# deeppowers/deeppowers

Measured on NVIDIA H100. Metric: ct_mult_relin_per_s, higher is better.
Workload: dtype u64

## Files before the change

deeppowers_b200/csrc/kernels.cu:

```cuda
#include <cooperative_groups.h>
#include <cuda.h>
#include <cuda_runtime.h>

#include <atomic>

#include "kernel_bodies.cuh"
#include "launch_util.hpp"

#ifndef DPFHE_PART
#define DPFHE_PART 0
#endif
#define DPFHE_PART_MAIN (DPFHE_PART == 0 || DPFHE_PART == 1)
#define DPFHE_PART_HYBRID (DPFHE_PART == 0 || DPFHE_PART == 2)
#define DPFHE_PART_GROUPED (DPFHE_PART == 0 || DPFHE_PART == 3)

namespace dpfhe {
namespace DPFHE_VNS {

__device__ __forceinline__ u32 ld_acquire_u32(const u32 *p) {
    u32 v;
    asm volatile("ld.acquire.gpu.global.u32 %0, [%1];" : "=r"(v) : "l"(p) : "memory");
    return v;
}
__device__ __forceinline__ void st_release_u32(u32 *p, u32 v) {
    asm volatile("st.release.gpu.global.u32 [%0], %1;" ::"l"(p), "r"(v) : "memory");
}
__device__ __forceinline__ u64 ld_acquire_u64(const u64 *p) {
    u64 v;
    asm volatile("ld.acquire.gpu.global.u64 %0, [%1];" : "=l"(v) : "l"(p) : "memory");
    return v;
}
__device__ __forceinline__ void st_release_u64(u64 *p, u64 v) {
    asm volatile("st.release.gpu.global.u64 [%0], %1;" ::"l"(p), "l"(v) : "memory");
}
__device__ __forceinline__ void spin_until(const u32 *flag, u32 tag) {
    while ((int)(ld_acquire_u32(flag) - tag) < 0) {
    }
}
__device__ __forceinline__ void wait_flags(const u32 *flags, u32 count, u32 tag) {
    if (threadIdx.x < count) spin_until(flags + threadIdx.x, tag);
    __syncthreads();
}
__device__ __forceinline__ void publish_flag(u32 *flag, u32 tag) {
    __threadfence();
    __syncthreads();
    if (threadIdx.x == 0) st_release_u32(flag, tag);
}
template <class Box>
__device__ __forceinline__ u32 draw_ticket(u32 *ticket, Box box, u32 tag, bool leader, bool post) {
    __shared__ u32 s_ct;
    if (threadIdx.x == 0) {
        u64 *const mb = box();
        if (leader) {
            const u32 t = atomicAdd(ticket, 1u);
            if (post) st_release_u64(mb, ((u64)tag << 32) | t);
            s_ct = t;
        } else {
            u64 m;
            do m = ld_acquire_u64(mb);
            while ((u32)(m >> 32) != tag);
            s_ct = (u32)m;
        }
    }
    __syncthreads();
    return s_ct;
}

template <int NT, bool PROF = false>
struct DevCta {
    unsigned long long *prof = nullptr;
    long long last = 0;
    unsigned long long t_start = 0, c_start = 0;
    __device__ __forceinline__ void prof_begin(unsigned long long *all) {
        if (PROF) {
            prof = all + (size_t)blockIdx.x * 16;
            last = clock64();
            c_start = (unsigned long long)last;
            asm volatile("mov.u64 %0, %%globaltimer;" : "=l"(t_start));
        }
    }
    __device__ __forceinline__ void prof_end() {
        if (PROF && threadIdx.x == 0) {
            unsigned long long t_end;
            asm volatile("mov.u64 %0, %%globaltimer;" : "=l"(t_end));
            prof[14] += t_end - t_start;
            prof[15] += (unsigned long long)clock64() - c_start;
        }
    }
    __device__ __forceinline__ void mark(int id) {
        if (PROF && threadIdx.x == 0) {
            const long long now = clock64();
            prof[id] += (unsigned long long)(now - last);
            last = now;
        }
    }
    template <class F>
    __device__ __forceinline__ void par(F f) {
        f((int)threadIdx.x);
        __syncthreads();
    }
    __device__ __forceinline__ void wait_ge(const u32 *flag, u32 target) { wait_flags(flag, 1, target); }
    template <class F>
    __device__ __forceinline__ void par_dom(F f) {
        f((int)threadIdx.x);
        if (NT <= 256) __syncthreads();
        else asm volatile("bar.sync %0, 256;" ::"r"(1 + ((int)threadIdx.x >> 8)) : "memory");
    }
    template <class F>
    __device__ __forceinline__ void par_warp(F f) {
        f((int)threadIdx.x);
        __syncwarp();
    }
};

#if DPFHE_PART_MAIN
template <int LOGN, int NT, int MINB, bool INVERSE>
__global__ void __launch_bounds__(NT, MINB) ntt_kernel(u64 *data, const Twiddle *__restrict__ tables,
                                                        const __grid_constant__ LimbTable lt, u32 L, size_t n_limbs) {
    extern __shared__ __align__(1024) unsigned char smem_raw[];
    u64 *buf = reinterpret_cast<u64 *>(smem_raw);
    constexpr size_t N = (size_t)1 << LOGN;
    DevCta<NT> cta;
    for (size_t w = blockIdx.x; w < n_limbs; w += gridDim.x) {
        const u32 l = (u32)(w % L);
        const LimbParams &p = lt.lp[l];
        if (INVERSE) ntt_inv_body<LOGN, NT>(cta, buf, data + w * N, tables + (size_t)l * N, p);
        else ntt_fwd_body<LOGN, NT>(cta, buf, data + w * N, tables + (size_t)l * N, p);
    }
}

__device__ __forceinline__ u32 smem_addr(const void *p) { return (u32)__cvta_generic_to_shared(p); }

template <int LOGN, int NT, int MINB>
__global__ void __launch_bounds__(NT, MINB) ntt_inv_tma_kernel(const __grid_constant__ CUtensorMap tm, u64 *data, const Twiddle *__restrict__ itw,
                                                                const __grid_constant__ LimbTable lt, u32 L) {
    extern __shared__ __align__(1024) unsigned char smem_raw[];
    __shared__ __align__(8) unsigned long long bar;
    u64 *buf = reinterpret_cast<u64 *>(smem_raw);
    constexpr size_t N = (size_t)1 << LOGN;
    constexpr int ROWS = (int)(N * 8 / 128), BOX_ROWS = ROWS < 256 ? ROWS : 256, BOXES = ROWS / BOX_ROWS;
    DevCta<NT> cta;
    const size_t w = blockIdx.x;
    const u32 l = (u32)(w % L);
    const u32 bar_a = smem_addr(&bar);
    if (threadIdx.x == 0) {
        asm volatile("mbarrier.init.shared::cta.b64 [%0], 1;" ::"r"(bar_a) : "memory");
        asm volatile("fence.mbarrier_init.release.cluster;" ::: "memory");
    }
    __syncthreads();
    if (threadIdx.x == 0) {
        asm volatile("mbarrier.arrive.expect_tx.shared::cta.b64 _, [%0], %1;" ::"r"(bar_a), "r"((u32)(N * 8)) : "memory");
#pragma unroll
        for (int b = 0; b < BOXES; ++b) {
            const int row = (int)(w * ROWS) + b * BOX_ROWS;
            asm volatile("cp.async.bulk.tensor.2d.shared::cluster.global.mbarrier::complete_tx::bytes [%0], [%1, {%2, %3}], [%4];"
                         ::"r"(smem_addr(smem_raw + (size_t)b * BOX_ROWS * 128)), "l"(reinterpret_cast<unsigned long long>(&tm)), "r"(0), "r"(row), "r"(bar_a)
                         : "memory");
        }
    }
    {
        u32 done = 0;
        while (!done) {
            asm volatile("{\n\t.reg .pred p;\n\tmbarrier.try_wait.parity.shared::cta.b64 p, [%1], 0;\n\tselp.u32 %0, 1, 0, p;\n\t}"
                         : "=r"(done)
                         : "r"(bar_a)
                         : "memory");
        }
    }
    ntt_inv_resident<LOGN, NT>(cta, buf, data + w * N, itw + (size_t)l * N, lt.lp[l]);
}

template <int NT, int MINB, bool INVERSE>
__global__ void __cluster_dims__(2, 1, 1) __launch_bounds__(NT, MINB)
    ntt_pair_kernel(u64 *data, const Twiddle *__restrict__ tables, const __grid_constant__ LimbTable lt, u32 L, size_t n_limbs) {
    extern __shared__ __align__(1024) unsigned char smem_raw[];
    u64 *buf = reinterpret_cast<u64 *>(smem_raw);
    constexpr size_t N = (size_t)1 << NTT_PAIR_LOGN;
    namespace cg = cooperative_groups;
    cg::cluster_group cluster = cg::this_cluster();
    const int h = (int)cluster.block_rank();
    const u64 *peer = cluster.map_shared_rank(buf, h ^ 1);
    DevCta<NT> cta;
    for (size_t w = blockIdx.x / 2; w < n_limbs; w += gridDim.x / 2) {
        const u32 l = (u32)(w % L);
        const LimbParams &p = lt.lp[l];
        const Twiddle *tw = tables + (size_t)l * N;
        if (!INVERSE) {
            ntt_fwd_half_load<NT>(cta, buf, data + w * N, tw, p, h);
            cluster.sync();
            ntt_fwd_half_finish<NT>(cta, buf, data + w * N, tw, p, h);
        } else {
            ntt_inv_half_passes<NT>(cta, buf, data + w * N, tw, p, h);
            cluster.sync();
            ntt_inv_half_outer<NT>(cta, buf, peer, data + w * N, tw, p, h);
            cluster.sync();
        }
    }
}

template <int LOGN, int NT, int MINB>
__global__ void __launch_bounds__(NT, MINB) ms_tau_kernel(const u64 *in, u64 *tau, const Twiddle *__restrict__ itw,
                                                           const __grid_constant__ LimbTable lt, const __grid_constant__ MsConsts K,
                                                           u32 L, size_t n_polys) {
    extern __shared__ __align__(1024) unsigned char smem_raw[];
    u64 *buf = reinterpret_cast<u64 *>(smem_raw);
    constexpr size_t N = (size_t)1 << LOGN;
    DevCta<NT> cta;
    const LimbParams &p = lt.lp[L - 1];
    for (size_t w = blockIdx.x; w < n_polys; w += gridDim.x)
        ms_tau_body<LOGN, NT>(cta, buf, in + (w * L + (L - 1)) * N, nullptr, itw + (size_t)(L - 1) * N, p, tau + w * N, K);
}

template <int LOGN, int NT, int MINB>
__global__ void __launch_bounds__(NT, MINB) ms_limb_kernel(const u64 *in, const u64 *tau, u64 *out, const Twiddle *__restrict__ tw,
                                                            const __grid_constant__ LimbTable lt, const __grid_constant__ MsConsts K,
                                                            u32 L, size_t n_items) {
    extern __shared__ __align__(1024) unsigned char smem_raw[];
    u64 *buf = reinterpret_cast<u64 *>(smem_raw);
    constexpr size_t N = (size_t)1 << LOGN;
    DevCta<NT> cta;
    const u32 Lo = L - 1;
    for (size_t w = blockIdx.x; w < n_items; w += gridDim.x) {
        const size_t poly = w / Lo;
        const u32 i = (u32)(w % Lo);
        ms_limb_body<LOGN, NT>(cta, buf, tau + poly * N, in + (poly * L + i) * N, out + (poly * Lo + i) * N, tw + (size_t)i * N, lt.lp[i], K, i);
    }
}

template <int LOGN, int NT, int MINB>
__global__ void __launch_bounds__(NT, MINB) md_tau_kernel(const u64 *in, u64 *tau, const Twiddle *__restrict__ itw, const __grid_constant__ MsConsts K,
                                                           const __grid_constant__ GroupConsts G, size_t n_items) {
    extern __shared__ __align__(1024) unsigned char smem_raw[];
    u64 *buf = reinterpret_cast<u64 *>(smem_raw);
    constexpr size_t N = (size_t)1 << LOGN;
    DevCta<NT> cta;
    const u32 L = G.Lq + G.K;
    for (size_t w = blockIdx.x; w < n_items; w += gridDim.x) {
        const size_t poly = w / G.K;
        const u32 s = G.Lq + (u32)(w % G.K);
        ms_tau_body<LOGN, NT>(cta, buf, in + (poly * L + s) * N, nullptr, itw + (size_t)s * N, G.lp_up[s], tau + w * N, K);
    }
}

template <int LOGN, int NT, int MINB>
__global__ void __launch_bounds__(NT, MINB) md_limb_kernel(const u64 *in, const u64 *tau, u64 *out, const Twiddle *__restrict__ tw,
                                                            const __grid_constant__ LimbTable lt, const __grid_constant__ MsConsts K,
                                                            const __grid_constant__ GroupConsts G, size_t n_items) {
    extern __shared__ __align__(1024) unsigned char smem_raw[];
    u64 *buf = reinterpret_cast<u64 *>(smem_raw);
    constexpr size_t N = (size_t)1 << LOGN;
    DevCta<NT> cta;
    const u32 Lq = G.Lq, L = Lq + G.K;
    for (size_t w = blockIdx.x; w < n_items; w += gridDim.x) {
        const size_t poly = w / Lq;
        const u32 i = (u32)(w % Lq);
        ms_limb_group<LOGN, NT, false>(cta, buf, tau + poly * G.K * N, N, in + (poly * L + i) * N, out + (poly * Lq + i) * N, tw + (size_t)i * N,
                                       lt.lp[i], K, G, i);
    }
}

template <int LOGN, int NT>
__global__ void __launch_bounds__(NT, 1) ckks_enc_fft_kernel(const Cplx *slots, double *coeffs, const Cplx *__restrict__ tw,
                                                              const u32 *__restrict__ tj, double sc) {
    extern __shared__ __align__(1024) unsigned char smem_raw[];
    constexpr size_t N = (size_t)1 << LOGN;
    DevCta<NT> cta;
    const size_t v = blockIdx.x;
    ckks_enc_fft_body<LOGN, NT>(cta, reinterpret_cast<Cplx *>(smem_raw), slots + v * (N / 2), coeffs + v * N, tw, tj, sc);
}

template <int LOGN, int NT, int MINB>
__global__ void __launch_bounds__(NT, MINB) ckks_enc_ntt_kernel(const double *coeffs, u64 *pt, const Twiddle *__restrict__ tw,
                                                                 const u64 *__restrict__ pow2, const __grid_constant__ LimbTable lt, u32 L) {
    extern __shared__ __align__(1024) unsigned char smem_raw[];
    u64 *buf = reinterpret_cast<u64 *>(smem_raw);
    constexpr size_t N = (size_t)1 << LOGN;
    DevCta<NT> cta;
    const size_t w = blockIdx.x;
    const u32 l = (u32)(w % L);
    const LimbParams &p = lt.lp[l];
    const double *x = coeffs + (w / L) * N;
    const u64 *p2 = pow2 + (size_t)l * CKKS_POW2_E;
    auto src = [&](int c) {
        U64x2 r;
        r.x = ckks_reduce(x[2 * c], p, p2);
        r.y = ckks_reduce(x[2 * c + 1], p, p2);
        return r;
    };
    ntt_fwd_src_body<LOGN, NT>(cta, buf, src, pt + w * N, tw + (size_t)l * N, p);
}

template <int NT, int MINB>
__global__ void __launch_bounds__(NT, MINB) ckks_enc_ntt_pair_kernel(const double *coeffs, u64 *pt, const Twiddle *__restrict__ tw,
                                                                      const u64 *__restrict__ pow2, const __grid_constant__ LimbTable lt, u32 L) {
    extern __shared__ __align__(1024) unsigned char smem_raw[];
    u64 *buf = reinterpret_cast<u64 *>(smem_raw);
    constexpr size_t N = (size_t)1 << NTT_PAIR_LOGN;
    DevCta<NT> cta;
    const size_t w = blockIdx.x / 2;
    const int h = (int)(blockIdx.x & 1);
    const u32 l = (u32)(w % L);
    const LimbParams &p = lt.lp[l];
    const double *x = coeffs + (w / L) * N;
    const u64 *p2 = pow2 + (size_t)l * CKKS_POW2_E;
    auto src = [&](int c) {
        U64x2 r;
        r.x = ckks_reduce(x[2 * c], p, p2);
        r.y = ckks_reduce(x[2 * c + 1], p, p2);
        return r;
    };
    ntt_fwd_half_load_src<NT>(cta, buf, src, tw + (size_t)l * N, p, h);
    ntt_fwd_half_finish<NT>(cta, buf, pt + w * N, tw + (size_t)l * N, p, h);
}

template <int LOGN, int NT>
__global__ void __launch_bounds__(NT, 1) ckks_dec_kernel(u64 *work, Cplx *slots, const Cplx *__restrict__ tw, const u32 *__restrict__ tj,
                                                          const __grid_constant__ LimbTable lt, const __grid_constant__ CkksConsts K, u32 L) {
    extern __shared__ __align__(1024) unsigned char smem_raw[];
    constexpr size_t N = (size_t)1 << LOGN;
    DevCta<NT> cta;
    const size_t v = blockIdx.x;
    ckks_dec_fft_body<LOGN, NT>(cta, reinterpret_cast<Cplx *>(smem_raw), work + v * L * N, slots + v * (N / 2), tw, tj, lt.lp, K, L);
}

template <int LOGN, int NT>
__global__ void __launch_bounds__(NT, 1) bgv_enc_kernel(const int64_t *slots, u32 *coeffs, const __grid_constant__ BgvTables T) {
    extern __shared__ __align__(1024) unsigned char smem_raw[];
    constexpr size_t N = (size_t)1 << LOGN;
    DevCta<NT> cta;
    const size_t v = blockIdx.x;
    bgv_enc_body<LOGN, NT>(cta, reinterpret_cast<u32 *>(smem_raw), slots + v * N, coeffs + v * N, T);
}

template <int LOGN, int NT, int MINB>
__global__ void __launch_bounds__(NT, MINB) bgv_enc_ntt_kernel(const u32 *coeffs, u64 *pt, const Twiddle *__restrict__ tw, u32 t,
                                                                const __grid_constant__ LimbTable lt, u32 L) {
    extern __shared__ __align__(1024) unsigned char smem_raw[];
    u64 *buf = reinterpret_cast<u64 *>(smem_raw);
    constexpr size_t N = (size_t)1 << LOGN;
    DevCta<NT> cta;
    const size_t w = blockIdx.x;
    const u32 l = (u32)(w % L);
    const LimbParams &p = lt.lp[l];
    const uint2 *x = reinterpret_cast<const uint2 *>(coeffs + (w / L) * N);
    auto src = [&](int c) {
        const uint2 v = x[c];
        U64x2 r;
        r.x = bgv_lift(v.x, t, p);
        r.y = bgv_lift(v.y, t, p);
        return r;
    };
    ntt_fwd_src_body<LOGN, NT>(cta, buf, src, pt + w * N, tw + (size_t)l * N, p);
}

template <int NT, int MINB>
__global__ void __launch_bounds__(NT, MINB) bgv_enc_ntt_pair_kernel(const u32 *coeffs, u64 *pt, const Twiddle *__restrict__ tw, u32 t,
                                                                     const __grid_constant__ LimbTable lt, u32 L) {
    extern __shared__ __align__(1024) unsigned char smem_raw[];
    u64 *buf = reinterpret_cast<u64 *>(smem_raw);
    constexpr size_t N = (size_t)1 << NTT_PAIR_LOGN;
    DevCta<NT> cta;
    const size_t w = blockIdx.x / 2;
    const int h = (int)(blockIdx.x & 1);
    const u32 l = (u32)(w % L);
    const LimbParams &p = lt.lp[l];
    const uint2 *x = reinterpret_cast<const uint2 *>(coeffs + (w / L) * N);
    auto src = [&](int c) {
        const uint2 v = x[c];
        U64x2 r;
        r.x = bgv_lift(v.x, t, p);
        r.y = bgv_lift(v.y, t, p);
        return r;
    };
    ntt_fwd_half_load_src<NT>(cta, buf, src, tw + (size_t)l * N, p, h);
    ntt_fwd_half_finish<NT>(cta, buf, pt + w * N, tw + (size_t)l * N, p, h);
}

template <int LOGN, int NT>
__global__ void __launch_bounds__(NT, 1) bgv_dec_kernel(u64 *work, u64 *slots, const __grid_constant__ BgvTables T, const __grid_constant__ LimbTable lt,
                                                         const __grid_constant__ BgvConsts K, u32 L) {
    extern __shared__ __align__(1024) unsigned char smem_raw[];
    constexpr size_t N = (size_t)1 << LOGN;
    DevCta<NT> cta;
    const size_t v = blockIdx.x;
    bgv_dec_body<LOGN, NT>(cta, reinterpret_cast<u32 *>(smem_raw), work + v * L * N, slots + v * N, T, lt.lp, K, L);
}

#endif
__device__ __forceinline__ void bulk_prefetch_l2(const void *p, u32 bytes) {
    asm volatile("cp.async.bulk.prefetch.L2.global [%0], %1;" ::"l"(p), "r"(bytes) : "memory");
}

#if DPFHE_PART_MAIN

template <int LOGN, int MODE>
__device__ __forceinline__ void prefetch_inputs(const KsArgs &A, size_t nc, size_t off, u32 bytes) {
    constexpr size_t N = (size_t)1 << LOGN;
    const size_t P = (size_t)A.L * N;
    if (MODE == KS_PLAIN) {
        bulk_prefetch_l2(A.a + nc * P + off, bytes);
    } else {
        bulk_prefetch_l2(A.a + nc * 2 * P + off, bytes);
        bulk_prefetch_l2(A.a + nc * 2 * P + P + off, bytes);
        if (MODE == KS_MUL_RELIN) {
            bulk_prefetch_l2(A.b + nc * 2 * P + off, bytes);
            bulk_prefetch_l2(A.b + nc * 2 * P + P + off, bytes);
        }
    }
}

template <int LOGN, int NT, int MODE, bool PROF, bool FILTER>
__device__ __forceinline__ void ks_fused_blk(const KsArgs &A, const LimbTable &lt, size_t batch, u32 *flags, u32 epoch, u32 *ticket, u64 *mail,
                                             unsigned long long *prof, u32 pf_dist) {
    extern __shared__ __align__(1024) unsigned char smem_raw[];
    constexpr size_t N = (size_t)1 << LOGN;
    constexpr u32 PAIR = (u32)ks_blk_pair<LOGN>();
    u64 *buf = reinterpret_cast<u64 *>(smem_raw);
    U64x2 *acc = reinterpret_cast<U64x2 *>(smem_raw + ((size_t)8 << KS_BLK_LOGN));
    DevCta<NT, PROF> cta;
    cta.prof_begin(prof);
    namespace cg = cooperative_groups;
    const u32 L = A.L, h = blockIdx.x % PAIR, slot = blockIdx.x / PAIR, i = slot % L, group = slot / L;
    const u64 *peer = buf;
    if constexpr (PAIR == 2) peer = cg::this_cluster().map_shared_rank(buf, (int)h ^ 1);
    auto pair_sync = [&]() {
        if constexpr (PAIR == 2) cg::this_cluster().sync();
        else __syncthreads();
    };
    const LimbParams &p = lt.lp[i];
    u32 executed = 0;
    for (u32 round = 0;; ++round) {
        if (FILTER) __syncthreads();
        const size_t ct = FILTER ? (size_t)round * (gridDim.x / (L * PAIR)) + group
                                 : (size_t)draw_ticket(ticket, [&] { return mail + group; }, epoch + round + 1, i == 0 && h == 0,
                                                       L * PAIR > 1);
        if (ct >= batch) break;
        if (FILTER && A.only[ct] == 0u) continue;
        if (pf_dist && threadIdx.x == 0 && ct + pf_dist < batch)
            prefetch_inputs<LOGN, MODE>(A, ct + pf_dist, (size_t)i * N + ((size_t)h << KS_BLK_LOGN), 8u << KS_BLK_LOGN);
        const u32 parity = (FILTER ? executed++ : round) & 1u;
        ks_blk_phase1_local<LOGN, NT, MODE>(cta, buf, acc, A, p, ct, i, (int)h);
        pair_sync();
        if (L > 1) {
            ks_blk_phase1_outer<LOGN, NT>(cta, buf, peer, A, p, i, (int)h, A.scratch + ((size_t)slot * 2 + parity) * N);
            __threadfence();
            pair_sync();
            if (h == 0 && threadIdx.x == 0) st_release_u32(flags + slot, epoch + round + 1);
            for (u32 jj = 1; jj < L; ++jj) {
                const u32 j = (i + jj) % L, sib = slot - i + j;
                wait_flags(flags + sib, 1, epoch + round + 1);
                cta.mark(3);
                ks_blk_phase2<LOGN, NT>(cta, buf, acc, A, p, ct, i, j, jj, (int)h, A.scratch + ((size_t)sib * 2 + parity) * N);
            }
        }
    }
    cta.prof_end();
}

template <int LOGN, int NT, int MINB, int MODE, bool PROF, bool FILTER = false>
__global__ void __launch_bounds__(NT, MINB) ks_fused_kernel(KsArgs A, const __grid_constant__ LimbTable lt, size_t batch, u32 *flags, u32 epoch,
                                                            u32 *ticket, u64 *mail, unsigned long long *prof, u32 pf_dist, u32 *consumed) {
    if constexpr (LOGN <= 13) {
        ks_fused_blk<LOGN, NT, MODE, PROF, FILTER>(A, lt, batch, flags, epoch, ticket, mail, prof, pf_dist);
    } else {
        extern __shared__ __align__(1024) unsigned char smem_raw[];
        constexpr size_t N = (size_t)1 << LOGN;
        u64 *buf = reinterpret_cast<u64 *>(smem_raw);
        DevCta<NT, PROF> cta;
        cta.prof_begin(prof);
        const u32 L = A.L, slot = blockIdx.x, i = slot % L, group = slot / L;
        const LimbParams &p = lt.lp[i];
        u32 executed = 0;
        __shared__ u32 s_base;
        if (consumed && threadIdx.x == 0) s_base = ld_acquire_u32(consumed + slot);
        __syncthreads();
        const u32 consumed_base = consumed ? s_base : 0u;
        u32 published = 0;
        for (u32 round = 0;; ++round) {
            if (FILTER) __syncthreads();
            const size_t ct = FILTER ? (size_t)round * (gridDim.x / L) + group
                                     : (size_t)draw_ticket(ticket, [&] { return mail + group; }, epoch + round + 1, i == 0, L > 1);
            if (ct >= batch) break;
            if (FILTER && A.only[ct] == 0u) continue;
            if (pf_dist && threadIdx.x == 0 && ct + pf_dist < batch) prefetch_inputs<LOGN, MODE>(A, ct + pf_dist, (size_t)i * N, (u32)(N * 8));
            const u32 parity = consumed ? 0u : (FILTER ? executed++ : round) & 1u;
            const size_t slot_stride = consumed ? 1 : 2;
            u64 *acc_rows = A.acc + (size_t)slot * 2 * N;
            ks_phase1<LOGN, NT, MODE>(cta, buf, A, p, ct, i, A.scratch + ((size_t)slot * slot_stride + parity) * N, acc_rows, 0, 0,
                                      consumed && L > 1 ? consumed + slot : nullptr, consumed_base + published * (L - 1));
            ++published;
            if (L > 1) {
                publish_flag(flags + slot, epoch + round + 1);
                for (u32 jj = 1; jj < L; ++jj) {
                    const u32 j = (i + jj) % L, sib = slot - i + j;
                    wait_flags(flags + sib, 1, epoch + round + 1);
                    cta.mark(3);
                    ks_phase2_digit<LOGN, NT>(cta, buf, A, p, ct, i, j, jj, A.scratch + ((size_t)sib * slot_stride + parity) * N, acc_rows);
                    if (consumed && threadIdx.x == 0) {
                        __threadfence();
                        atomicAdd(consumed + sib, 1u);
                    }
                }
            }
        }
        cta.prof_end();
    }
}

template <int LOGN, int NT, int MINB>
__global__ void __launch_bounds__(NT, MINB) ks_hoist_kernel(HoistArgs A, const __grid_constant__ LimbTable lt, size_t batch, u32 *flags, u32 epoch,
                                                            u32 *ticket, u64 *mail) {
    extern __shared__ __align__(1024) unsigned char smem_raw[];
    constexpr size_t N = (size_t)1 << LOGN;
    u64 *buf = reinterpret_cast<u64 *>(smem_raw);
    DevCta<NT> cta;
    const u32 L = A.L, slot = blockIdx.x, i = slot % L, group = slot / L;
    const LimbParams &p = lt.lp[i];
    for (u32 round = 0;; ++round) {
        const u32 tag = epoch + round + 1;
        const size_t ct = draw_ticket(ticket, [&] { return mail + group; }, tag, i == 0, true);
        if (ct >= batch) break;
        const u32 parity = round & 1u;
        hoist_phase1<LOGN, NT>(cta, buf, A, p, ct, i, A.scratch + ((size_t)slot * 2 + parity) * N);
        publish_flag(flags + slot, tag);
        for (u32 jj = 1; jj < L; ++jj) {
            const u32 j = (i + jj) % L, sib = slot - i + j;
            wait_flags(flags + sib, 1, tag);
            hoist_phase2<LOGN, NT>(cta, buf, A, p, ct, i, j, A.scratch + ((size_t)sib * 2 + parity) * N);
        }
    }
}

template <int LOGN, int NT, int MINB, int ROT_CB, bool PF>
__global__ void __launch_bounds__(NT, MINB) rot_apply_kernel(RotApplyArgs A, const __grid_constant__ LimbTable lt, size_t batch, u32 nseg) {
    DevCta<NT> cta;
    constexpr int NC = 1 << (LOGN - 1);
    const size_t n_blocks = (batch + ROT_CB - 1) / ROT_CB, n_items = n_blocks * A.L * nseg;
    const int seg_chunks = NC / (int)nseg;
    for (size_t w = blockIdx.x; w < n_items; w += gridDim.x) {
        const u32 seg = (u32)(w % nseg), i = (u32)((w / nseg) % A.L);
        const size_t ct0 = (w / nseg / A.L) * ROT_CB;
        const u32 n_ct = (u32)(batch - ct0 < (size_t)ROT_CB ? batch - ct0 : (size_t)ROT_CB);
        rot_apply_rows<LOGN, NT, ROT_CB, PF>(cta, A, lt.lp[i], ct0, n_ct, i, (int)seg * seg_chunks, ((int)seg + 1) * seg_chunks);
    }
}

template <int LOGN>
__global__ void __launch_bounds__(256) negmask_kernel(u64 *mask, u32 g, u32 L) {
    constexpr u32 N = 1u << LOGN;
    for (u32 k = blockIdx.x * blockDim.x + threadIdx.x; k < N; k += gridDim.x * blockDim.x) {
        const u32 e = (k * g) & (2 * N - 1);
        const u64 v = e >= N ? 1ull : 0ull;
        for (u32 l = 0; l < L; ++l) mask[(size_t)l * N + (e & (N - 1))] = v;
    }
}

template <int LOGN>
__global__ void __launch_bounds__(256) kprime_kernel(const u64 *__restrict__ key, const u64 *__restrict__ M, const u64 *__restrict__ delta,
                                                     u64 *__restrict__ out, const LimbParams *__restrict__ lps, u32 L) {
    constexpr size_t N = (size_t)1 << LOGN;
    const size_t P = (size_t)L * N, total = 2 * P;
    for (size_t e = (size_t)blockIdx.x * blockDim.x + threadIdx.x; e < total; e += (size_t)gridDim.x * blockDim.x) {
        const u32 c = (u32)(e / P), i = (u32)((e % P) / N);
        const size_t n = e % N;
        const LimbParams p = lps[i];
        u64 s = 0;
        for (u32 j = 0; j < L; ++j) {
            if (j == i) continue;
            s = csub(s + mulmod(key[((size_t)j * 2 + c) * P + (size_t)i * N + n], delta[j * L + i], p), p.q);
        }
        out[e] = mulmod(s, M[(size_t)i * N + n], p);
    }
}

#endif
#if DPFHE_PART_HYBRID
template <int LOGN, int NT, int MODE, bool LV>
__device__ __forceinline__ void ks_hybrid_body(const KsArgs &A, const LimbTable &lt, const MsConsts &K, size_t batch, u32 *flags, u32 epoch,
                                               u32 *ticket, u64 *mail) {
    extern __shared__ __align__(1024) unsigned char smem_raw[];
    constexpr size_t N = (size_t)1 << LOGN;
    u64 *buf = reinterpret_cast<u64 *>(smem_raw);
    DevCta<NT> cta;
    const u32 L = A.L, GS = L + 1, slot = blockIdx.x, i = slot % GS, group = slot / GS, base = slot - i;
    const u32 key_shift = LV ? A.Lk - GS : 0u;
    const bool special = i == L;
    const LimbParams &p = lt.lp[i];
    u64 *hyb = A.hyb + (size_t)group * KS_HYB_ROWS * N;
    auto acc_of = [&](u32 parity) { return A.acc + ((size_t)slot * 2 + parity) * 2 * N; };
    auto divide = [&](size_t ct, u32 tag, u32 parity) {
        wait_flags(flags + (base + L), 1, tag);
        const size_t P = (size_t)L * N;
        for (u32 c = 0; c < 2; ++c) {
            u64 *row = A.out + ct * 2 * P + c * P + (size_t)i * N;
            ms_limb_body<LOGN, NT, true>(cta, buf, hyb + ks_hyb_tau_row(parity, c) * N, acc_of(parity) + c * N, row, A.tw + (size_t)i * N, p, K, i);
        }
    };
    bool pending = false;
    size_t prev_ct = 0;
    u32 prev_tag = 0, prev_parity = 0;
    for (u32 round = 0;; ++round) {
        const u32 tag = epoch + round + 1, parity = round & 1u;
        const size_t ct = draw_ticket(ticket, [&] { return mail + (size_t)group * 2 + parity; }, tag, i == 0, true);
        if (ct >= batch) break;
        if (!special) {
            if constexpr (LV)
                ks_phase1<LOGN, NT, MODE, true, true>(cta, buf, A, p, ct, i, A.scratch + ((size_t)slot * 2 + parity) * N, acc_of(parity), K.qlm[i],
                                                      K.qlm_s[i], nullptr, 0, ~0u, nullptr, key_shift);
            else
                ks_phase1<LOGN, NT, MODE, true>(cta, buf, A, p, ct, i, A.scratch + ((size_t)slot * 2 + parity) * N, acc_of(parity), K.qlm[i], K.qlm_s[i]);
            publish_flag(flags + slot, tag);
            for (u32 jj = 1; jj < L; ++jj) {
                const u32 j = (i + jj) % L;
                wait_flags(flags + (base + j), 1, tag);
                ks_phase2_digit<LOGN, NT, true, false, LV>(cta, buf, A, p, ct, i, j, jj, A.scratch + ((size_t)(base + j) * 2 + parity) * N, acc_of(parity),
                                                           key_shift);
            }
            if (pending) divide(prev_ct, prev_tag, prev_parity);
            pending = true;
            prev_ct = ct;
            prev_tag = tag;
            prev_parity = parity;
        } else {
            for (u32 jj = 0; jj < L; ++jj) {
                const u32 j = (group + jj) % L;
                wait_flags(flags + (base + j), 1, tag);
                ks_phase2_digit<LOGN, NT, true, true, LV>(cta, buf, A, p, ct, i, j, jj, A.scratch + ((size_t)(base + j) * 2 + parity) * N, hyb, key_shift);
            }
            for (u32 c = 0; c < 2; ++c)
                ms_tau_body<LOGN, NT, true>(cta, buf, hyb + c * N, hyb + c * N, A.itw + (size_t)i * N, p, hyb + ks_hyb_tau_row(parity, c) * N, K);
            publish_flag(flags + slot, tag);
        }
    }
    if (pending) divide(prev_ct, prev_tag, prev_parity);
}

template <int LOGN, int NT, int MINB, int MODE>
__global__ void __launch_bounds__(NT, MINB) ks_hybrid_kernel(KsArgs A, const __grid_constant__ LimbTable lt, const __grid_constant__ MsConsts K,
                                                             size_t batch, u32 *flags, u32 epoch, u32 *ticket, u64 *mail) {
    ks_hybrid_body<LOGN, NT, MODE, false>(A, lt, K, batch, flags, epoch, ticket, mail);
}

template <int LOGN, int NT, int MINB, int MODE>
__global__ void __launch_bounds__(NT, MINB) ks_hybrid_level_kernel(KsArgs A, const __grid_constant__ LimbTable lt, const __grid_constant__ MsConsts K,
                                                                   size_t batch, u32 *flags, u32 epoch, u32 *ticket, u64 *mail) {
    ks_hybrid_body<LOGN, NT, MODE, true>(A, lt, K, batch, flags, epoch, ticket, mail);
}

#endif
#if DPFHE_PART_GROUPED
template <int LOGN, int NT, int MODE, bool ADD, bool RS = false, bool LV = false>
__device__ __forceinline__ void ks_grouped_body(const KsArgs &A, const LimbTable &lt, const MsConsts &K, const GroupConsts &G, size_t batch, u32 *flags,
                                                u32 epoch, u32 *ticket, u64 *mail, const u64 *addend, const DotArgs *dot,
                                                const RescaleConsts *R = nullptr) {
    static_assert(!ADD || MODE == KS_ROTATE, "the fused addition is a Horner step of rotations");
    static_assert(!RS || (!ADD && (MODE == KS_MUL_RELIN || MODE == KS_DOT)), "multiply-and-rescale follows a product");
    extern __shared__ __align__(1024) unsigned char smem_raw[];
    constexpr size_t N = (size_t)1 << LOGN;
    u64 *buf = reinterpret_cast<u64 *>(smem_raw);
    DevCta<NT> cta;
    const u32 Lq = G.Lq, Ks = G.K, dnum = G.dnum, GS = Lq + Ks, slot = blockIdx.x, i = slot % GS, group = slot / GS, base = slot - i;
    const u32 key_shift = LV ? A.Lk - GS : 0u;
    const bool special = i >= Lq;
    const LimbParams &p = lt.lp[i];
    auto hyb_of = [&](u32 k) { return A.hyb + ((size_t)group * Ks + k) * KS_HYB_ROWS * N; };
    auto acc_of = [&](u32 parity) { return A.acc + ((size_t)slot * 2 + parity) * 2 * N; };
    auto drop_of = [&](u32 parity, u32 c) { return R->tau + (((size_t)group * 2 + parity) * 2 + c) * N; };
    auto divide = [&](size_t ct, u32 tag, u32 parity) {
        if constexpr (RS) if (threadIdx.x == 0) spin_until(R->tau_flag + group, tag);
        wait_flags(flags + (base + Lq), Ks, tag);
        if constexpr (RS) {
            const size_t P = (size_t)(Lq - 1) * N;
            for (u32 c = 0; c < 2; ++c)
                ms_limb_group<LOGN, NT, true, false, true>(cta, buf, hyb_of(0) + ks_hyb_tau_row(parity, c) * N, (size_t)KS_HYB_ROWS * N, acc_of(parity) + c * N,
                                                           A.out + ct * 2 * P + c * P + (size_t)i * N, A.tw + (size_t)i * N, p, K, G, i, nullptr,
                                                           drop_of(parity, c), R);
            return;
        }
        const size_t P = (size_t)Lq * N;
        for (u32 c = 0; c < 2; ++c) {
            u64 *row = A.out + ct * 2 * P + c * P + (size_t)i * N;
            const u64 *add_row = nullptr;
            if constexpr (ADD) add_row = addend + ct * 2 * P + c * P + (size_t)i * N;
            ms_limb_group<LOGN, NT, true, ADD>(cta, buf, hyb_of(0) + ks_hyb_tau_row(parity, c) * N, (size_t)KS_HYB_ROWS * N, acc_of(parity) + c * N, row,
                                               A.tw + (size_t)i * N, p, K, G, i, add_row);
        }
    };
    bool pending = false;
    size_t prev_ct = 0;
    u32 prev_tag = 0, prev_parity = 0;
    for (u32 round = 0;; ++round) {
        const u32 tag = epoch + round + 1, parity = round & 1u;
        const size_t ct = draw_ticket(ticket, [&] { return mail + (size_t)group * 2 + parity; }, tag, i == 0, true);
        if (ct >= batch) break;
        const u64 *t_rows = A.scratch + ((size_t)base * 2 + parity) * N;
        if (!special) {
            const u32 g_own = i / Ks;
            ks_phase1<LOGN, NT, MODE, true, LV>(cta, buf, A, G.lp_up[i], ct, i, A.scratch + ((size_t)slot * 2 + parity) * N, acc_of(parity), K.qlm[i],
                                                K.qlm_s[i], nullptr, 0, g_own, dot, key_shift);
            publish_flag(flags + slot, tag);
            for (u32 jj = 1; jj < dnum; ++jj) {
                const u32 g = (g_own + jj) % dnum, lo = g * Ks, cnt = lo + Ks < Lq ? Ks : Lq - lo;
                wait_flags(flags + (base + lo), cnt, tag);
                ks_phase2_group<LOGN, NT, false, LV>(cta, buf, A, G, p, ct, i, g, jj, t_rows, 2 * N, acc_of(parity), key_shift);
            }
            if constexpr (RS) if (i == Lq - 1) {
                const u32 lo = g_own * Ks;
                wait_flags(flags + (base + lo), i - lo, tag);
                for (u32 c = 0; c < 2; ++c)
                    ms_tau_body<LOGN, NT, true>(cta, buf, acc_of(parity) + c * N, acc_of(parity) + c * N, A.itw + (size_t)i * N, R->lp_drop,
                                                drop_of(parity, c), K);
                publish_flag(R->tau_flag + group, tag);
                continue;
            }
            if (pending) divide(prev_ct, prev_tag, prev_parity);
            pending = true;
            prev_ct = ct;
            prev_tag = tag;
            prev_parity = parity;
        } else {
            u64 *hyb = hyb_of(i - Lq);
            for (u32 jj = 0; jj < dnum; ++jj) {
                const u32 g = (group + jj) % dnum, lo = g * Ks, cnt = lo + Ks < Lq ? Ks : Lq - lo;
                wait_flags(flags + (base + lo), cnt, tag);
                ks_phase2_group<LOGN, NT, true, LV>(cta, buf, A, G, p, ct, i, g, jj, t_rows, 2 * N, hyb, key_shift);
            }
            for (u32 c = 0; c < 2; ++c)
                ms_tau_body<LOGN, NT, true>(cta, buf, hyb + c * N, hyb + c * N, A.itw + (size_t)i * N, G.lp_up[i], hyb + ks_hyb_tau_row(parity, c) * N, K);
            publish_flag(flags + slot, tag);
        }
    }
    if (pending) divide(prev_ct, prev_tag, prev_parity);
}

template <int LOGN, int NT, int MINB, int MODE, bool ADD = false>
__global__ void __launch_bounds__(NT, MINB) ks_grouped_kernel(KsArgs A, const __grid_constant__ LimbTable lt, const __grid_constant__ MsConsts K,
                                                              const __grid_constant__ GroupConsts G, size_t batch, u32 *flags, u32 epoch,
                                                              u32 *ticket, u64 *mail, const u64 *addend) {
    ks_grouped_body<LOGN, NT, MODE, ADD>(A, lt, K, G, batch, flags, epoch, ticket, mail, addend, nullptr);
}

template <int LOGN, int NT, int MINB, int MODE>
__global__ void __launch_bounds__(NT, MINB) ks_rescale_grouped_kernel(KsArgs A, const __grid_constant__ LimbTable lt, const __grid_constant__ MsConsts K,
                                                                      const __grid_constant__ GroupConsts G, const __grid_constant__ DotArgs D,
                                                                      const __grid_constant__ RescaleConsts R, size_t batch, u32 *flags, u32 epoch,
                                                                      u32 *ticket, u64 *mail) {
    ks_grouped_body<LOGN, NT, MODE, false, true>(A, lt, K, G, batch, flags, epoch, ticket, mail, nullptr, MODE == KS_DOT ? &D : nullptr, &R);
}

template <int LOGN, int NT, int MINB, int MODE, bool RS>
__global__ void __launch_bounds__(NT, MINB) ks_level_grouped_kernel(KsArgs A, const __grid_constant__ LimbTable lt, const __grid_constant__ MsConsts K,
                                                                    const __grid_constant__ GroupConsts G, const __grid_constant__ DotArgs D,
                                                                    const __grid_constant__ RescaleConsts R, size_t batch, u32 *flags, u32 epoch,
// ... 1002 lines not shown
```

Measured before the change: 516,400.

## Consume sibling limbs in readiness order with split cluster barrier

```diff
diff --git a/deeppowers_b200/csrc/kernels.cu b/deeppowers_b200/csrc/kernels.cu
--- a/deeppowers_b200/csrc/kernels.cu
+++ b/deeppowers_b200/csrc/kernels.cu
@@ -33,10 +33,12 @@
 __device__ __forceinline__ void st_release_u64(u64 *p, u64 v) {
     asm volatile("st.release.gpu.global.u64 [%0], %1;" ::"l"(p), "l"(v) : "memory");
 }
+__device__ __forceinline__ bool round_reached(u32 v, u32 tag) { return (int)(v - tag) >= 0; }
 __device__ __forceinline__ void spin_until(const u32 *flag, u32 tag) {
-    while ((int)(ld_acquire_u32(flag) - tag) < 0) {
-    }
-}
+    while (!round_reached(ld_acquire_u32(flag), tag)) {
+    }
+}
+__device__ __forceinline__ bool flag_ready(const u32 *flag, u32 tag) { return round_reached(ld_acquire_u32(flag), tag); }
 __device__ __forceinline__ void wait_flags(const u32 *flags, u32 count, u32 tag) {
     if (threadIdx.x < count) spin_until(flags + threadIdx.x, tag);
     __syncthreads();
@@ -409,6 +411,20 @@
     }
 }
 
+
+template <u32 PAIR>
+__device__ __forceinline__ u32 pick_sibling(const u32 *gflags, u32 i, u32 L, u32 left, u32 tag) {
+    static_assert(PAIR * 16 <= 32, "one lane per producer CTA of every sibling (L <= 16, LimbTable)");
+    const u32 lane = threadIdx.x, k = lane / PAIR, j = i + k < L ? i + k : i + k - L;
+    const u32 *f = gflags + j * PAIR + lane % PAIR;
+    const bool up = k < L && (left >> k & 1u) && flag_ready(f, tag);
+    const u32 ready = __ballot_sync(~0u, up);
+    const u32 whole = PAIR == 2 ? ready & (ready >> 1) & 0x55555555u : ready;
+    const u32 kb = whole ? (u32)(__ffs(whole) - 1) / PAIR : (u32)__ffs(left) - 1;
+    if (k == kb && !up) spin_until(f, tag);
+    return kb;
+}
+
 template <int LOGN, int NT, int MODE, bool PROF, bool FILTER>
 __device__ __forceinline__ void ks_fused_blk(const KsArgs &A, const LimbTable &lt, size_t batch, u32 *flags, u32 epoch, u32 *ticket, u64 *mail,
                                              unsigned long long *prof, u32 pf_dist) {
@@ -428,6 +444,7 @@
         else __syncthreads();
     };
     const LimbParams &p = lt.lp[i];
+    __shared__ u32 s_left, s_pick;
     u32 executed = 0;
     for (u32 round = 0;; ++round) {
         if (FILTER) __syncthreads();
@@ -443,12 +460,20 @@
         pair_sync();
         if (L > 1) {
             ks_blk_phase1_outer<LOGN, NT>(cta, buf, peer, A, p, i, (int)h, A.scratch + ((size_t)slot * 2 + parity) * N);
-            __threadfence();
-            pair_sync();
-            if (h == 0 && threadIdx.x == 0) st_release_u32(flags + slot, epoch + round + 1);
+            publish_flag(flags + blockIdx.x, epoch + round + 1);
+            if constexpr (PAIR == 2) cg::this_cluster().barrier_arrive();
             for (u32 jj = 1; jj < L; ++jj) {
-                const u32 j = (i + jj) % L, sib = slot - i + j;
-                wait_flags(flags + sib, 1, epoch + round + 1);
+                if (threadIdx.x < 32) {
+                    const u32 left = jj == 1 ? (1u << L) - 2u : s_left;
+                    const u32 k = pick_sibling<PAIR>(flags + (size_t)(slot - i) * PAIR, i, L, left, epoch + round + 1);
+                    if (threadIdx.x == 0) {
+                        s_left = left & ~(1u << k);
+                        s_pick = k;
+                    }
+                }
+                __syncthreads();
+                const u32 j = i + s_pick < L ? i + s_pick : i + s_pick - L, sib = slot - i + j;
+                if constexpr (PAIR == 2) if (jj == 1) cg::this_cluster().barrier_wait();
                 cta.mark(3);
                 ks_blk_phase2<LOGN, NT>(cta, buf, acc, A, p, ct, i, j, jj, (int)h, A.scratch + ((size_t)sib * 2 + parity) * N);
             }
```

Measured after the change: 519,700 (median of 6 runs). No clear change (+0.6%).
